# DeepakSridhar/fgdm

Measured on AMD Instinct MI355X. Metric: 512x512 images/sec @ 50 DDIM steps, seg-ControlNet+CFG, higher is better.
Workload: dtype f16

## Files before the change

### fgdm_amd/_lib.py

```python
import ctypes as C
import os

HERE = os.path.dirname(os.path.abspath(__file__))
LIB_PATH = os.path.join(HERE, 'libfgdm_hip.so')

MAX_LEVELS = 8
MAX_CONTROLNETS = 4

FLAG_USE_ORIGINAL = 1
FLAG_ONLY_MID_CONTROL = 2
FLAG_NO_CONTROL = 4
FLAG_CFG_PAIRS = 8

ACT_NONE, ACT_SILU, ACT_RELU, ACT_GEGLU, ACT_QGELU = 0, 1, 2, 3, 4
OUT_F16, OUT_F32, OUT_F32_NCHW, OUT_F16_T = 0, 1, 2, 3
STRIDE2_PAD_BR = -2


class FgdmConfig(C.Structure):
    _fields_ = [
        ('in_channels', C.c_int32), ('out_channels', C.c_int32), ('model_channels', C.c_int32),
        ('num_res_blocks', C.c_int32), ('n_levels', C.c_int32), ('channel_mult', C.c_int32 * MAX_LEVELS),
        ('n_attention_resolutions', C.c_int32), ('attention_resolutions', C.c_int32 * MAX_LEVELS),
        ('num_heads', C.c_int32), ('context_dim', C.c_int32), ('use_adapter', C.c_int32),
# ... 38 lines not shown
    'fgdm_controlnet': (_i, [_p, _i, _p, _p, _p, _i, _i, _i, _p, _i64, _p]),
    'fgdm_ddim_step': (_i, [_p, _p, _p, _f, _f, _f, _f, _f, _p, _p, _p, _p, _i64, _p]),
    'fgdm_plms_combine': (_i, [_p, _p, _p, _p, _i, _p, _i64, _p]),
    'fgdm_axpby': (_i, [_p, _f, _p, _f, _p, _i64, _p]),
    'fgdm_mask_blend': (_i, [_p, _p, _p, _p, _i64, _p]),
    'fgdm_ancestral_step': (_i, [_p, _p, _f, _f, _f, _f, _f, _p, _p, _i64, _p]),
    'fgdm_sample_ddim': (_i, [_p, _p, _p, _p, _f, _i, C.POINTER(_i64), C.POINTER(_f), C.POINTER(_f), C.POINTER(_f),
                              _p, _i, _i, _i, _i, _p]),
    'fgdm_profile_begin': (_i, [_p, _i]),
    'fgdm_profile_end': (_i, [_p, C.POINTER(C.c_double)]),
    'fgdm_workspace_stats': (_i, [_p, C.POINTER(_i64), C.POINTER(_i64)]),
    'fgdm_launch_stats': (_i, [_p, C.POINTER(_i64), C.POINTER(_i64), C.POINTER(_i64)]),
    'fgdm_op_conv2d': (_i, [_p, _i, _p, _i, _p, _p, _p, _p, _i, _i, _i, _i, _i, _i, _i, _i, _f, _p, _p]),
    'fgdm_op_linear': (_i, [_p, _p, _p, _p, _i, _i, _i, _i, _i, _i, _i, _p, _p]),
    'fgdm_debug_force_igemm_cfg': (_i, [_i]),
    'fgdm_bench_igemm': (_i, [_i] * 13 + [C.POINTER(_f)]),
    'fgdm_op_linear_ln_linear': (_i, [_p] * 8 + [_i] * 5 + [_p, _p, C.POINTER(_i), _p]),
    'fgdm_bench_norm': (_i, [_i] * 7 + [C.POINTER(_f)]),
    'fgdm_bench_attention': (_i, [_i] * 6 + [C.POINTER(_f)]),
    'fgdm_bench_ff': (_i, [_i] * 4 + [C.POINTER(_f)]),
    'fgdm_op_groupnorm': (_i, [_p, _i, _p, _i, _i, _i, _p, _p, _f, _i, _p, _p]),
    'fgdm_op_layernorm': (_i, [_p, _i, _i, _p, _p, _f, _p, _p]),
    'fgdm_op_attention': (_i, [_p, _i, _p, _i, _p, _i, _p, _i, _i, _i, _i, _i, _i, _p]),
    'fgdm_op_attention_ex': (_i, [_p, _i, _p, _i, _p, _i, _p, _i, _i, _i, _i, _i, _i, _i, _p]),
    'fgdm_debug_last_attention_kernel': (_i, []),
    'fgdm_op_small_attention': (_i, [_p, _i, _i, _i, _p, _i, _i, _i, _i, _i, _i, _p]),
    'fgdm_op_vae_attention': (_i, [_p, _p, _p, _p, _i, _i, _i, _p]),
    'fgdm_op_softmax_rows': (_i, [_p, _p, _i, _i, _p]),
    'fgdm_op_nchw_to_nhwc': (_i, [_p, _p, _i, _i, _i, _i, _p]),
    'fgdm_op_nhwc_to_nchw': (_i, [_p, _p, _i, _i, _i, _p]),
# ... 29 lines not shown
```

### fgdm_amd/csrc/common.h

```cpp
#pragma once
#include <hip/hip_runtime.h>
#include <stdint.h>

typedef _Float16 half_t;
typedef _Float16 h8 __attribute__((ext_vector_type(8)));
typedef _Float16 h4 __attribute__((ext_vector_type(4)));
typedef _Float16 h2 __attribute__((ext_vector_type(2)));
typedef float f32x16 __attribute__((ext_vector_type(16)));
typedef float f32x4 __attribute__((ext_vector_type(4)));

__device__ __forceinline__ float gelu_f(float x) {
    const float z = fminf(fabsf(x), 6.0f);
    float p = -4.7132482596e-04f;
    p = __builtin_fmaf(p, z, 7.0652551839e-03f);
    p = __builtin_fmaf(p, z, -5.1762067461e-02f);
    p = __builtin_fmaf(p, z, -4.6008771426e-01f);
    p = __builtin_fmaf(p, z, -1.1507295505e+00f);
    p = __builtin_fmaf(p, z, -4.8959157159e-05f - 1.0f);
    const float t = __builtin_amdgcn_exp2f(p);
    return __builtin_fmaf(fabsf(x), 0.5f - t, 0.5f * x);
}

typedef float f32x2 __attribute__((ext_vector_type(2)));
__device__ __forceinline__ f32x2 gelu2_f(f32x2 x) {
// ... 34 lines not shown
    void* out;
    const half_t* zero;
    int C0, C1;
    int B, H, W;
    int Ho, Wo;
    int M, N;
    int K;
    int mode, act, out_kind;
    int ld_out, ld_res;
    int rv_stride;
    int rows_per_sample;
    float scale;
    int force_cfg;
    int splitk;
    float* ws;
    int debug;
    const float* ln_stats;
    const float* ln_u;
    int ln_slots;
    float ln_eps;
    float* stats_out;
    void* out2;
    int split_n, out_kind2, ld_out2;
};

int igemm_launch(const IgemmArgs& a, hipStream_t s);
void igemm_set_force_cfg(int cfg);
void igemm_set_twin_layers(bool on);
void igemm_set_pair_hint(int mult);
int igemm2_launch(const IgemmArgs& a, int cfg, hipStream_t s);
int igemm_stats_slots(const IgemmArgs& a);
int row_stats_slots(int C);
int row_stats_launch(const half_t* x, int rows, int C, float* stats , hipStream_t s);
int igemm_splitk_factor(const IgemmArgs& a);
int igemm_splitk_reduce(const IgemmArgs& a, hipStream_t s);
size_t igemm_npad(int n);

#define GN_PIX_PER_CHUNK 256
void groupnorm_set_group(bool on);
int groupnorm_launch(const half_t* x0, int C0, const half_t* x1, int C1, int B, int HW,
                     const float* gamma, const float* beta, float eps, int silu,
                     half_t* out, float* ws , hipStream_t s);
size_t groupnorm_ws_floats(int B, int HW);
int layernorm_launch(const half_t* x, int rows, int C, const float* gamma, const float* beta, float eps,
                     half_t* out, hipStream_t s);

int attention_launch(const half_t* Q, int ldq, const half_t* K, int ldk, const half_t* Vt, int ldvt,
                     half_t* O, int ldo, int B, int H, int T, int Tk, int d, int q_prescaled, hipStream_t s);
int attention_last_kernel();

// ... 71 lines not shown
```

### fgdm_amd/csrc/engine.hip

```cpp
#include "engine_shared.h"
#include "knobs.h"

#include <algorithm>
#include <array>
#include <cmath>
#include <cstdlib>
#include <cstdio>
#include <cstring>
#include <map>
#include <memory>
#include <string>
#include <unordered_map>
#include <vector>

namespace {

struct Arena {
    struct Blk { char* p; size_t sz; bool free; };
    std::vector<std::vector<Blk>> slabs;
    std::vector<char*> bases;
    size_t slab_bytes = (size_t)4 << 30;
    size_t in_use = 0, peak = 0;
    bool scoped = false;
    std::vector<void*> live;
// ... 240 lines not shown
    std::unordered_map<std::string, ParamSlot> params;
    Net unet;
    std::vector<Net> cns;
    Vae vae;
    Clip clip;
    struct CtxKV { Tensor k, vt; };
    std::unordered_map<const Layer*, CtxKV> ctx_cache;
    int ctx_B = 0, ctx_T = 0;
    int ctx_tokens = 77;
    Arena arena;
    half_t* zero = nullptr;
    std::unordered_map<std::string, std::vector<void*>> weight_allocs;
    std::unordered_map<std::string, bool> comp_dirty, comp_packed;
    std::string cur_comp;
    bool ln_fold = true;
    hipStream_t s = nullptr;
    std::vector<std::unique_ptr<Arena>> cn_arena;
    Arena* ar = &arena;
    hipStream_t s2 = nullptr;
    hipEvent_t ev_fork = nullptr, ev_join = nullptr;
    bool twin_streams = false;
    bool pair_launch = true;
    int group_max = FGDM_MAX_GROUP;
    bool gn_group = true;
    long paired_launches = 0, replayed_launches = 0, paired_problems = 0;
    struct Deferred { const GemmW* w; Tensor src; int idx; float scale; Arena* owner; };
    Prof prof;

    int fail(int code, const std::string& m) { err = m; return code; }

// ... 656 lines not shown
        a.mode = mode; a.act = e.act; a.out_kind = e.out_kind;
        const int nout = e.act == ACT_GEGLU ? w.N / 2 : w.N;
        a.out = e.out ? e.out : (void*)out->p;
        a.ld_out = e.ld_out ? e.ld_out : nout;
        a.rows_per_sample = e.rps ? e.rps : Ho * Wo;
        a.scale = e.scale;
        a.out2 = e.out2; a.out_kind2 = e.out_kind2; a.ld_out2 = e.ld_out2; a.split_n = e.split_n;
        const int taps = mode == IG_LINEAR ? 1 : 9;
        if (taps * (a.C0 + a.C1) != a.K) return fail(FGDM_ERR_ARG, "gemm: K mismatch");
        if (!a.out) return fail(FGDM_ERR_NOMEM, "gemm: null output (workspace exhausted?)");
        char tag[56] = "";
        if (prof.on) snprintf(tag, sizeof(tag), "igemm M%d N%d K%d mode%d act%d out%d l%ds%dr%dv%d", a.M, a.N, a.K, a.mode, a.act, a.out_kind,
                              e.ln ? 1 : 0, e.stats ? 1 : 0, e.resid ? 1 : 0, e.rowvec ? 1 : 0);
        a.splitk = igemm_splitk_factor(a);
        if (a.splitk > 1) {
            a.ws = (float*)ar->alloc((size_t)a.splitk * a.M * a.N * sizeof(float));
            if (!a.ws) return fail(FGDM_ERR_NOMEM, "workspace (split-K partials)");
        }
        if (e.ln) {
            if (!w.ln_u || !e.ln->p || a.splitk > 1) return fail(FGDM_ERR_STATE, "gemm: LayerNorm fold without folded weights / statistics");
            a.ln_stats = e.ln->p; a.ln_slots = e.ln->slots; a.ln_u = w.ln_u; a.ln_eps = w.ln_eps;
        } else if (w.ln_u) {
            return fail(FGDM_ERR_STATE, "gemm: these weights have a LayerNorm folded in; statistics are required");
        }
        if (e.stats) {
            e.stats->slots = igemm_stats_slots(a);
            e.stats->p = (float*)ar->alloc((size_t)a.M * std::max(e.stats->slots, row_stats_slots(nout)) * 2 * sizeof(float));
            if (!e.stats->p) return fail(FGDM_ERR_NOMEM, "workspace (LayerNorm statistics)");
            if (e.stats->slots) a.stats_out = e.stats->p;
        }
        double nbytes = 0.0;
// ... 993 lines not shown
    for (auto& a : e->cn_arena) a->end_scope(rc != FGDM_OK);
    return rc;
}

extern "C" {

static std::string g_create_err;

int fgdm_create(const fgdm_config* cfg, int device, fgdm_engine** out) {
    if (!cfg || !out) return FGDM_ERR_ARG;
    fgdm_engine* e = nullptr;
    int rc = make_desc(cfg, &e);
    if (rc != FGDM_OK) { g_create_err = "unsupported configuration"; return rc; }
    e->device = device;
    e->ln_fold = knob_on(KNOB_LN_FOLD);
    rc = e->ensure_device();
    if (rc != FGDM_OK) {
        g_create_err = e->err + " [" + hipGetErrorString(hipGetLastError()) + "]";
        delete e;
        return rc;
    }
    e->twin_streams = knob_on(KNOB_TWIN_STREAMS);
    e->pair_launch = knob_on(KNOB_PAIR_LAUNCH);
    e->group_max = std::max(2, std::min(FGDM_MAX_GROUP, knob_int(KNOB_GROUP_MAX)));
    e->gn_group = knob_on(KNOB_GN_GROUP);
    if (e->twin_streams && !e->cns.empty()) {
        if (hipStreamCreateWithFlags(&e->s2, hipStreamNonBlocking) != hipSuccess ||
            hipEventCreateWithFlags(&e->ev_fork, hipEventDisableTiming) != hipSuccess ||
            hipEventCreateWithFlags(&e->ev_join, hipEventDisableTiming) != hipSuccess) {
            g_create_err = "second stream could not be created";
// ... 318 lines not shown
```

### fgdm_amd/csrc/engine_shared.h

```cpp
#pragma once
#include "common.h"
#include "../../include/fgdm.h"

#include <algorithm>
#include <cmath>
#include <vector>

static int roundup(int x, int m) { return (x + m - 1) / m * m; }

static std::vector<int> conv3_kmap(int Cin, int* cin_pad) {
    const bool implicit = (Cin % 64) == 0;
    const int cp = implicit ? Cin : roundup(Cin, Cin % 8 == 0 ? 8 : 4);
    const int K = implicit ? 9 * Cin : roundup(9 * cp, 64);
    std::vector<int> kmap(K, -1);
    for (int tap = 0; tap < 9; ++tap)
        for (int c = 0; c < Cin; ++c) {
            const int k = implicit ? ((c >> 6) * 9 + tap) * 64 + (c & 63) : tap * cp + c;
            kmap[k] = c * 9 + tap;
        }
    *cin_pad = cp;
    return kmap;
}

template <class After, class Gemm>
// ... 27 lines not shown
    ~TmpDev() { for (void* p : ptrs) (void)hipFree(p); }
    template <typename T> T* alloc(size_t n) {
        T* d = nullptr;
        if (hipMalloc(&d, n * sizeof(T)) != hipSuccess) return nullptr;
        ptrs.push_back(d);
        return d;
    }
    template <typename T> T* up(const std::vector<T>& h) {
        T* d = alloc<T>(std::max<size_t>(h.size(), 256 / sizeof(T)));
        if (d) (void)hipMemcpy(d, h.data(), h.size() * sizeof(T), hipMemcpyHostToDevice);
        return d;
    }
};
static int plan_splitk(IgemmArgs& a, TmpDev& tmp) {
    a.splitk = igemm_splitk_factor(a);
    if (a.splitk > 1 && !(a.ws = tmp.alloc<float>((size_t)a.splitk * a.M * a.N))) return FGDM_ERR_NOMEM;
    return FGDM_OK;
}
inline half_t* g_zero_page() {
    static half_t* z = nullptr;
    if (!z) { if (hipMalloc(&z, 4096) != hipSuccess) return nullptr; (void)hipMemset(z, 0, 4096); }
    return z;
}
```

### fgdm_amd/csrc/igemm.hip

```cpp
#include "common.h"
#include "knobs.h"
#include <algorithm>

#define LDS_AS __attribute__((address_space(3)))
#define GLB_AS __attribute__((address_space(1)))

__device__ __forceinline__ void glds16(const void* g, void* lds_wave_base) {
    __builtin_amdgcn_global_load_lds((const GLB_AS void*)g, (LDS_AS void*)lds_wave_base, 16, 0, 0);
}


__device__ __forceinline__ float ln_scale(float acc, float mean, float rstd, float u) {
    float t, w;
    asm("v_fma_f32 %0, %1, %2, %3" : "=v"(t) : "v"(-mean), "v"(u), "v"(acc));
    asm("v_mul_f32 %0, %1, %2" : "=v"(w) : "v"(rstd), "v"(t));
    return w;
}

template <int BM, int BN, int WM, int WN>
__global__ __launch_bounds__(WM * WN * 64) void igemm_kernel(const IgemmArgs a) {
    constexpr int T = WM * WN * 64;
    constexpr int TM = BM / WM, TN = BN / WN;
    constexpr int MI = TM / 32, NI = TN / 32;
    constexpr int A_IT = BM * 8 / T, B_IT = BN * 8 / T;
// ... 291 lines not shown
            else if (a.N == 128 && rows >= 192) force = 10;
        }
    }
    return force;
}

int igemm_stats_slots(const IgemmArgs& a) {
    if (a.out_kind != OUT_F16 || a.act == ACT_GEGLU || a.splitk > 1 || (a.N % 320) || (a.K & 31) || (a.C0 & 31) || (a.C1 & 31)) return 0;
    const int f = pick_force(a);
    if (f < 4) return 0;
    const int tile = (f - 4) & 15;
    const bool stats64 = knob_once(KNOB_IGEMM_STATS64) != 0;
    return (tile == 0 || tile == 2 || tile == 3 || tile == 5 || (tile == 7 && stats64)) ? a.N / 160 : 0;
}

int igemm_launch(const IgemmArgs& a, hipStream_t s) {
    if (a.M <= 0 || a.N <= 0 || a.K <= 0 || (a.K & 63) || (a.C0 & 63) || (a.C1 & 63)) return FGDM_ERR_ARG;
    if (a.act == ACT_GEGLU && (a.N & 63)) return FGDM_ERR_ARG;
    if (a.ln_stats && (a.mode != IG_LINEAR || a.C1 || a.ln_slots <= 0 || !a.ln_u)) return FGDM_ERR_ARG;
    if (a.stats_out && igemm_stats_slots(a) == 0) return FGDM_ERR_ARG;
    if (a.out2 && (a.act == ACT_GEGLU || a.splitk > 1 || a.stats_out || a.split_n <= 0 || a.split_n >= a.N || (a.split_n % 640))) return FGDM_ERR_ARG;
    if (a.splitk > 1) {
        if (!a.ws || a.ln_stats) return FGDM_ERR_ARG;
        const bool fat = (long)((a.M + 255) / 256) * (a.N / 320) * a.splitk >= 192 && !(a.K & 31) && !(a.C0 & 31) && !(a.C1 & 31);
        const int rc = igemm2_launch(a, fat ? 0 : 2, s);
        return rc == FGDM_OK ? igemm_splitk_reduce(a, s) : rc;
    }
    int force = pick_force(a);
    const bool mfma32 = knob_once(KNOB_IGEMM_MFMA32) != 0;
    if (mfma32 && force >= 4 && force <= 6 && !a.force_cfg && !g_force_cfg) force += 3;
    if (force >= 4) return igemm2_launch(a, force - 4, s);
    struct Cfg { int bm, bn; float eff; int per_cu; };
    static const Cfg cfgs[] = {{128, 128, 1.00f, 2}, {128, 64, 0.80f, 3}, {64, 64, 0.62f, 4}};
    int best = 0;
    float best_cost = 1e30f;
    for (int i = 0; i < 3; ++i) {
        const Cfg& c = cfgs[i];
        const long nblk = (long)((a.M + c.bm - 1) / c.bm) * ((a.N + c.bn - 1) / c.bn);
        const long slots = 256L * c.per_cu;
        const float rounds = (float)((nblk + slots - 1) / slots);
        const long conc = std::min<long>(c.per_cu, (nblk + 255) / 256);
// ... 13 lines not shown
```

### fgdm_amd/csrc/igemm2.hip

```cpp
#include "common.h"
#include "knobs.h"
#include <algorithm>
#include <type_traits>

#pragma clang diagnostic ignored "-Winline-asm"
#define LDS_AS __attribute__((address_space(3)))
#define GLB_AS __attribute__((address_space(1)))

namespace {

__device__ __forceinline__ void glds16(const void* g, unsigned lds_wave_addr) {
    unsigned keep;
    asm volatile("s_mov_b32 %0, m0\n\ts_mov_b32 m0, %2\n\ts_nop 0\n\tglobal_load_lds_dwordx4 %1, off\n\ts_mov_b32 m0, %0"
                 : "=&s"(keep)
                 : "v"(g), "s"(lds_wave_addr)
                 : "memory", "m0");
}
__device__ __forceinline__ void glds16_m0(const void* g, unsigned lds_wave_addr) {
    asm volatile("s_mov_b32 m0, %1\n\ts_nop 0\n\tglobal_load_lds_dwordx4 %0, off" ::"v"(g), "s"(lds_wave_addr) : "memory", "m0");
}
__device__ __forceinline__ void glds16_sv(unsigned voff, const void* sbase, unsigned lds_wave_addr) {
    asm volatile("s_mov_b32 m0, %2\n\ts_nop 0\n\tglobal_load_lds_dwordx4 %0, %1" ::"v"(voff), "s"(sbase), "s"(lds_wave_addr) : "memory", "m0");
}
__device__ __forceinline__ unsigned lds_addr(const void* p) { return (unsigned)(size_t)(LDS_AS const void*)p; }
// ... 479 lines not shown
            step(std::true_type{}, kt + 1, xb, xa);
        }
        if (kt < nr) {
            step(std::true_type{}, kt, xa, xb);
            ++kt;
#pragma unroll
            for (int i = 0; i < MI; ++i) xa[i] = xb[i];
        }
        if (kt < nk) step(std::false_type{}, kt, xa, xb);
        if (kt + 1 < nk) step(std::false_type{}, kt + 1, xb, xa);
        if (kt + 2 < nk) step(std::false_type{}, kt + 2, xa, xb);
        wait_vmcnt<0>();
    }

    if constexpr (SPLIT) {
        float* wsp = a.ws + (size_t)split * a.M * a.N;
#pragma unroll
        for (int i = 0; i < MI; ++i) {
            const int row = m0 + wm * TM + i * MS + lrow;
            if (row >= a.M) continue;
#pragma unroll
            for (int j = 0; j < NI; ++j)
#pragma unroll
                for (int g = 0; g < AR / 4; ++g) {
                    const int col = n0 + wn * TN + j * MS + (MS == 32 ? 8 * g : 0) + lq;
                    f32x4 pk = {acc[j][i][g * 4], acc[j][i][g * 4 + 1], acc[j][i][g * 4 + 2], acc[j][i][g * 4 + 3]};
                    *(f32x4*)(wsp + (size_t)row * a.N + col) = pk;
                }
        }
        return;
// ... 516 lines not shown
        const bool staged = LN && a.out_kind2 == OUT_F16_T && a.rows_per_sample % 32 == 0 && a.M % 32 == 0 && a.ld_out2 % 8 == 0 &&
                            ((size_t)a.out2 & 15) == 0;
        if (!staged || a.rowvec) return 0;
    }
    if (!a.rowvec) return 1;
    return (BM - 1) / a.rows_per_sample + 2 <= RV_MAX ? 2 : 0;
}
template <int BM, int BN, int WM, int WN, int STAGES, bool CONV, bool GEGLU, bool SPLIT, int MS, bool LN, bool FAST, int PIPE>
int launch2(const IgemmArgs& a, hipStream_t s) {
    const bool fast_on = knob_once(KNOB_IGEMM_EPI_PATHS) != 0;
    if constexpr (FAST && !SPLIT && !LN) {
        if (a.debug)
            return epilogue_path<BM, GEGLU, LN>(a) == 1 ? launch2p<BM, BN, WM, WN, STAGES, CONV, GEGLU, SPLIT, MS, LN, 1, (PIPE == 2 ? 1 : PIPE), true>(a, s)
                                                        : FGDM_ERR_ARG;
    }
    if (a.debug) return FGDM_ERR_ARG;
    if constexpr (SPLIT) return launch2p<BM, BN, WM, WN, STAGES, CONV, GEGLU, SPLIT, MS, LN, 0, PIPE, false>(a, s);
    if constexpr (FAST && !SPLIT) {
        switch (fast_on ? epilogue_path<BM, GEGLU, LN>(a) : 0) {
            case 1: return launch2p<BM, BN, WM, WN, STAGES, CONV, GEGLU, SPLIT, MS, LN, 1, PIPE, false>(a, s);
            case 2: if constexpr (!GEGLU && !LN) return launch2p<BM, BN, WM, WN, STAGES, CONV, GEGLU, SPLIT, MS, LN, 2, PIPE, false>(a, s);
            default: break;
        }
    }
    return launch2p<BM, BN, WM, WN, STAGES, CONV, GEGLU, SPLIT, MS, LN, 0, 0, false>(a, s);
}
template <int BM, int BN, bool GEGLU, int MS, int PIPE, int WM, int WN>
int launch2m(const IgemmArgs& a, hipStream_t s) {
    constexpr int PL = PIPE == 2 ? 1 : PIPE;
    return a.mode == IG_LINEAR ? launch2<BM, BN, WM, WN, 4, false, GEGLU, false, MS, false, MS == 16, PL>(a, s)
// ... 3 lines not shown
int launch2ln(const IgemmArgs& a, hipStream_t s) {
    return launch2<BM, BN, WM, WN, 4, false, GEGLU, false, MS, true, MS == 16, (PIPE == 2 ? 1 : PIPE)>(a, s);
}
template <int BM, int BN, int MS, int PIPE, int WM = 4, int WN = 2>
int launch_tile(const IgemmArgs& a, hipStream_t s) {
    const bool g = a.act == ACT_GEGLU;
    if (a.ln_stats) {
        if constexpr (BN == 256) { if (g) return launch2ln<BM, BN, true, MS, PIPE, WM, WN>(a, s); }
        if constexpr (BN == 128) return FGDM_ERR_ARG;
        else return launch2ln<BM, BN, false, MS, PIPE, WM, WN>(a, s);
    }
    if constexpr (BN == 256) { if (g) return launch2m<BM, BN, true, MS, PIPE, WM, WN>(a, s); }
    return launch2m<BM, BN, false, MS, PIPE, WM, WN>(a, s);
}

__global__ __launch_bounds__(256) void splitk_reduce_kernel(const IgemmArgs a) {
    const size_t total4 = (size_t)a.M * a.N / 4, plane = (size_t)a.M * a.N;
    for (size_t i = (size_t)blockIdx.x * 256 + threadIdx.x; i < total4; i += (size_t)gridDim.x * 256) {
        const size_t e0 = i * 4;
        const int row = (int)(e0 / a.N), col = (int)(e0 - (size_t)row * a.N);
        f32x4 v = *(const f32x4*)(a.ws + e0);
        for (int s = 1; s < a.splitk; ++s) {
            const f32x4 u = *(const f32x4*)(a.ws + (size_t)s * plane + e0);
            v[0] += u[0]; v[1] += u[1]; v[2] += u[2]; v[3] += u[3];
        }
        h4 r = {(half_t)0, (half_t)0, (half_t)0, (half_t)0};
        if (a.resid) r = *(const h4*)(a.resid + (size_t)row * a.ld_res + col);
        h4 o;
#pragma unroll
        for (int e = 0; e < 4; ++e) {
            float x = v[e] + (a.bias ? a.bias[col + e] : 0.f);
            if (a.rowvec) x += a.rowvec[(size_t)(row / a.rows_per_sample) * a.rv_stride + col + e];
            if (a.act == ACT_SILU) x = silu_f(x);
            else if (a.act == ACT_RELU) x = fmaxf(x, 0.f);
            else if (a.act == ACT_QGELU) x = silu_f(x, 1.702f);
            const half_t y = (half_t)(x * a.scale);
            o[e] = a.resid ? (half_t)((float)y + (float)r[e]) : y;
        }
        *(h4*)((half_t*)a.out + (size_t)row * a.ld_out + col) = o;
    }
}

}

static thread_local bool g_twin_layers = false;
void igemm_set_twin_layers(bool on) { g_twin_layers = on; }

int igemm_splitk_factor(const IgemmArgs& a) {
    if (a.force_cfg || a.act == ACT_GEGLU || a.out_kind != OUT_F16 || a.N % 320 || (a.K & 31)) return 1;
    const int nk = a.K >> 5;
    const bool fat = knob_once(KNOB_SPLITK_FAT) != 0;
    if (fat && a.rows_per_sample > 64 && a.rows_per_sample <= 256 && (nk >= 540 || (nk >= 360 && !g_twin_layers))) return 2;
    if (a.rows_per_sample > 64 || nk < 96) return 1;
    return (fat && nk >= 360) ? 8 : 4;
}
int igemm_splitk_reduce(const IgemmArgs& a, hipStream_t s) {
    const size_t total4 = (size_t)a.M * a.N / 4;
    const int grid = (int)std::min<size_t>(2048, (total4 + 255) / 256);
    FGDM_LAUNCH(splitk_reduce_kernel, dim3(grid), dim3(256), 0, s, a);
    return hipGetLastError() == hipSuccess ? FGDM_OK : FGDM_ERR_HIP;
}

static bool halo_geometry(const IgemmArgs& a) {
    if (a.mode != IG_CONV3 || a.Ho != a.H || a.Wo != a.W || (a.C0 & 63) || (a.C1 & 63) || (a.K % 288) || a.debug) return false;
    if ((a.W == 16 || a.W == 32 || a.W == 64) && (a.H * a.W) % 256 == 0) return true;
    return a.W == 8 && a.H == 8;
}

int igemm2_launch(const IgemmArgs& a, int cfg, hipStream_t s) {
    if ((a.K & 31) || (a.C0 & 31) || (a.C1 & 31)) return FGDM_ERR_ARG;
    const int pipe_default = knob_once(KNOB_IGEMM_PIPE);
    const int tile = cfg & 15, psel = cfg >> 4;
    const size_t px = a.mode == IG_LINEAR ? (size_t)a.M : (size_t)a.B * a.H * a.W;
    const bool small = px * (size_t)std::max(a.C0, a.C1) * 2 < (1ull << 32) && (size_t)(a.N + 320) * a.K * 2 < (1ull << 32);
    const bool pipe = (psel == 0 ? pipe_default != 0 : psel == 2) && small;
    const bool halo = knob_once(KNOB_IGEMM_HALO) != 0 && pipe && halo_geometry(a);
    const int bn = (tile == 1 || tile == 4) ? 256 : tile == 6 ? 128 : tile == 7 ? 160 : 320;
    if (a.N % bn) return FGDM_ERR_ARG;
    if (a.act == ACT_GEGLU && bn != 256) return FGDM_ERR_ARG;
    if (a.splitk > 1) {
        if ((tile != 2 && tile != 0) || a.ln_stats) return FGDM_ERR_ARG;
        const int nk_all = a.K >> 5;
        if (halo && nk_all % a.splitk == 0 && (nk_all / a.splitk) % 9 == 0)
            return tile == 0 ? launch2<256, 320, 4, 2, 4, true, false, true, 16, false, false, 2>(a, s)
                             : launch2<128, 320, 4, 2, 4, true, false, true, 16, false, false, 2>(a, s);
        if (tile == 0 && pipe)
            return a.mode == IG_LINEAR ? launch2<256, 320, 4, 2, 4, false, false, true, 16, false, false, 1>(a, s)
                                       : launch2<256, 320, 4, 2, 4, true, false, true, 16, false, false, 1>(a, s);
        if (pipe)
            return a.mode == IG_LINEAR ? launch2<128, 320, 4, 2, 4, false, false, true, 16, false, false, 1>(a, s)
                                       : launch2<128, 320, 4, 2, 4, true, false, true, 16, false, false, 1>(a, s);
        return a.mode == IG_LINEAR ? launch2<128, 320, 4, 2, 4, false, false, true, 16, false, false, 0>(a, s)
                                   : launch2<128, 320, 4, 2, 4, true, false, true, 16, false, false, 0>(a, s);
    }
    if (a.ln_stats && a.mode != IG_LINEAR) return FGDM_ERR_ARG;
    const int persist_mode = knob_once(KNOB_IGEMM_PERSIST);
    const bool persist_on = persist_mode != 0;
    if (persist_on && tile == 1 && pipe && a.act == ACT_GEGLU && a.mode == IG_LINEAR && !a.C1 && a.out_kind == OUT_F16 && !a.rowvec &&
// ... 17 lines not shown
```

### fgdm_amd/csrc/knobs.h

```cpp
#pragma once
#include "common.h"
#include <array>
#include <cstdlib>

#define FGDM_STR_(x) #x
#define FGDM_STR(x) FGDM_STR_(x)

#define FGDM_KNOBS(X)                                                                                                          \
    X(ATTN_PP, "FGDM_ATTN_PP", "1", "0: the four-wave attention kernel where the eight-wave ping-pong one would run")           \
    X(ATTN_DQ, "FGDM_ATTN_DQ", "3", "long self-attention, d = 40: 3 = two-strand kernel, 32-wide V^T P^T; 1 = 16-wide; 0 = off") \
    X(ATTN_DQ80, "FGDM_ATTN_DQ80", "1", "0: the ping-pong kernel instead of the two-strand one at d = 80")                      \
    X(ATTN_ABL, "FGDM_ATTN_ABL", "0", "ablation instantiations of the two-strand kernel (tools/bench_attention.py only)")       \
    X(ATTN_CROSS, "FGDM_ATTN_CROSS", "4", "query chunks per wave of the text-token kernel (65 - 96 keys); 0 = off")             \
    X(ATTN_CROSS_LONG, "FGDM_ATTN_CROSS_LONG", "8", "query chunks per wave of the key-resident kernel (97 - 256 keys); 0 = off") \
    X(IGEMM_EPI_PATHS, "FGDM_IGEMM_EPI_PATHS", "1", "0: the general GEMM epilogue instead of the host-selected straight-line paths") \
    X(IGEMM_HALO, "FGDM_IGEMM_HALO", "1", "0: per-tap K loop instead of the halo-tile loop (stride-1 3x3 convolutions, split K too)") \
    X(IGEMM_MFMA32, "FGDM_IGEMM_MFMA32", "0", "1: automatic tile choices take the 32x32x16 MFMA instantiations")                \
    X(IGEMM_OTHER_WIDTHS, "FGDM_IGEMM_OTHER_WIDTHS", "1", "0: widths 128 / 256 / 512 back on the 2-stage kernel")               \
    X(IGEMM_PERSIST, "FGDM_IGEMM_PERSIST", "1", "GEGLU projections: 1 = persistent, tiles round-robin; 2 = contiguous runs; 0 = off") \
    X(IGEMM_PIPE, "FGDM_IGEMM_PIPE", "1", "0: the phase-locked K loop instead of the software-pipelined one")                   \
    X(IGEMM_SMALL_M, "FGDM_IGEMM_SMALL_M", "1", "0: linears with a thin 128-row grid stay on 128 x 320 tiles")                  \
    X(IGEMM_SMALL_TILES, "FGDM_IGEMM_SMALL_TILES", "1", "0: the 8x8 level's linears back on the 2-stage kernel")                \
    X(IGEMM_STATS64, "FGDM_IGEMM_STATS64", "1", "0: the 64 x 160 tile leaves the LayerNorm partial sums to the row-statistics pass") \
    X(SPLITK_FAT, "FGDM_SPLITK_FAT", "1", "0: split K four ways on 128 x 320 tiles at the 8x8 level only")                      \
    X(PAIR_FAT_TILES, "FGDM_PAIR_FAT_TILES", "1", "0: grouped launches keep the tile a single problem would take")              \
    X(GN_REG, "FGDM_GN_REG", "1024", "largest pixel count per sample of the register-resident GroupNorm; 0 = off")              \
    X(GN_REG_NG, "FGDM_GN_REG_NG", "4", "widest slice of the register-resident GroupNorm, in groups")                           \
    X(GN_FUSED_MAXKB, "FGDM_GN_FUSED_MAXKB", "64", "largest LDS slice (KB) of the single-kernel GroupNorm; 0 = always two kernels") \
    X(GN_CHUNK, "FGDM_GN_CHUNK", FGDM_STR(GN_PIX_PER_CHUNK), "pixels per partial-sum chunk of the two-kernel GroupNorm (multiples of 64)") \
    X(LN_FOLD, "FGDM_LN_FOLD", "1", "fgdm_create; 0: the transformer blocks' LayerNorms as kernels of their own")               \
    X(TWIN_STREAMS, "FGDM_TWIN_STREAMS", "0", "fgdm_create; 1: the ControlNets on a second stream next to the UNet encoder")    \
    X(PAIR_LAUNCH, "FGDM_PAIR_LAUNCH", "1", "fgdm_create; 0: no grouped launches of twin layers")                               \
    X(GROUP_MAX, "FGDM_GROUP_MAX", FGDM_STR(FGDM_MAX_GROUP), "fgdm_create; problems per grouped launch, clamped to [2, FGDM_MAX_GROUP]") \
    X(GN_GROUP, "FGDM_GN_GROUP", "1", "fgdm_create; 0: single-pass GroupNorm launches stay out of the grouped launches")        \
    X(PAIR_DEBUG, "FGDM_PAIR_DEBUG", nullptr, "set (to anything): fgdm_destroy prints how many replayed launches were fused")   \
    X(PROF_DUMP, "FGDM_PROF_DUMP", nullptr, "path: fgdm_profile_end writes the per-shape time table there")                     \
    X(BENCH_DATA_SCALE, "FGDM_BENCH_DATA_SCALE", "1", "atof; scale of the random operands of fgdm_bench_igemm / _attention")

enum Knob {
// ... 28 lines not shown
```

### fgdm_amd/csrc/ops_abi.hip

```cpp
#include "engine_shared.h"

static int op_pack(IgemmArgs& a, TmpDev& tmp, const float* w, const float* bias, int N, int K, int Ks, bool geglu,
                   const int* kmap = nullptr, const float* gamma = nullptr, const float* beta = nullptr) {
    auto host = [](const float* d, size_t n, std::vector<float>& v) { v.resize(n); return hipMemcpy(v.data(), d, n * sizeof(float), hipMemcpyDefault) == hipSuccess; };
    std::vector<float> wh, bh(N, 0.f), g, bt;
    if (!host(w, (size_t)N * Ks, wh) || (bias && !host(bias, N, bh))) return FGDM_ERR_HIP;
    if (gamma && (!host(gamma, K, g) || !host(beta, K, bt))) return FGDM_ERR_HIP;
    const size_t npad = igemm_npad(N);
    std::vector<half_t> pk(npad * (size_t)K, (half_t)0);
    std::vector<float> bp(npad, 0.f), u(gamma ? npad : 0, 0.f);
    for (int pr = 0; pr < N; ++pr) {
        int sr = pr;
        if (geglu) { const int grp = pr >> 6, within = pr & 63; sr = within < 32 ? grp * 32 + within : N / 2 + grp * 32 + (within - 32); }
        const float* row = &wh[(size_t)sr * Ks];
        double us = 0.0, cs = 0.0;
        for (int k = 0; k < K; ++k) {
            const int ks = kmap ? kmap[k] : k;
            if (ks < 0) continue;
            const half_t wq = (half_t)(gamma ? row[ks] * g[k] : row[ks]);
            pk[(size_t)pr * K + k] = wq;
            if (gamma) { us += (double)(float)wq; cs += (double)bt[k] * (double)row[ks]; }
        }
        bp[pr] = gamma ? (float)((double)bh[sr] + cs) : bh[sr];
        if (gamma) u[pr] = (float)us;
// ... 123 lines not shown
    rc = igemm_launch(a, s);
    if (rc == FGDM_OK && !slots) { slots = row_stats_slots(C); rc = row_stats_launch((const half_t*)h_out, M, C, stats, s); }
    if (slots_used) *slots_used = a.stats_out ? slots : -slots;
    if (rc != FGDM_OK) { (void)hipStreamSynchronize(s); return rc; }
    b.A0 = (const half_t*)h_out; b.C0 = C; b.zero = a.zero;
    b.ln_stats = stats; b.ln_slots = slots; b.ln_eps = 1e-5f;
    const int nout = act2 == ACT_GEGLU ? N2 / 2 : N2;
    b.B = 1; b.H = 1; b.W = M; b.Ho = 1; b.Wo = M; b.M = M; b.N = N2; b.K = C; b.mode = IG_LINEAR; b.act = act2;
    b.out_kind = OUT_F16; b.out = y_out; b.ld_out = nout; b.rows_per_sample = M; b.scale = 1.f;
    rc = igemm_launch(b, s);
    (void)hipStreamSynchronize(s);
    return rc;
}

int fgdm_debug_force_igemm_cfg(int cfg) { igemm_set_force_cfg(cfg); return FGDM_OK; }

int fgdm_op_groupnorm(const void* x0, int C0, const void* x1, int C1, int B, int HW, const float* gamma, const float* beta,
                      float eps, int silu, void* out, void* stream) {
    if (!x0 || !gamma || !beta || !out) return FGDM_ERR_ARG;
    hipStream_t s = as_stream(stream);
    float* ws = nullptr;
    if (hipMalloc(&ws, groupnorm_ws_floats(B, HW) * sizeof(float)) != hipSuccess) return FGDM_ERR_NOMEM;
    const int rc = groupnorm_launch((const half_t*)x0, C0, (const half_t*)x1, C1, B, HW, gamma, beta, eps, silu, (half_t*)out, ws, s);
    (void)hipStreamSynchronize(s);
    (void)hipFree(ws);
    return rc;
}
int fgdm_op_layernorm(const void* x, int rows, int C, const float* gamma, const float* beta, float eps, void* out, void* stream) {
    if (!x || !gamma || !beta || !out) return FGDM_ERR_ARG;
    return layernorm_launch((const half_t*)x, rows, C, gamma, beta, eps, (half_t*)out, as_stream(stream));
// ... 67 lines not shown
```

### include/fgdm.h

```cpp
#ifndef FGDM_H
#define FGDM_H
#include <stdint.h>
#ifdef __cplusplus
extern "C" {
#endif

#define FGDM_MAX_LEVELS 8
#define FGDM_MAX_CONTROLNETS 4

typedef struct fgdm_engine fgdm_engine;

typedef struct fgdm_config {
    int32_t in_channels, out_channels, model_channels, num_res_blocks;
    int32_t n_levels;
    int32_t channel_mult[FGDM_MAX_LEVELS];
    int32_t n_attention_resolutions;
    int32_t attention_resolutions[FGDM_MAX_LEVELS];
    int32_t num_heads, context_dim;
    int32_t use_adapter;
    int32_t n_controlnets;
    int32_t hint_channels;
    int64_t workspace_bytes;
    int32_t vae_ch, vae_n_levels;
    int32_t vae_ch_mult[FGDM_MAX_LEVELS];
// ... 69 lines not shown
int fgdm_profile_begin(fgdm_engine* e, int stride );
int fgdm_profile_end(fgdm_engine* e, double* out);
int fgdm_workspace_stats(fgdm_engine* e, int64_t* peak_bytes, int64_t* reserved_bytes);
int fgdm_launch_stats(fgdm_engine* e, int64_t* replayed_launches, int64_t* fused_launches, int64_t* fused_problems);

#define FGDM_STRIDE2_PAD_BR (-2)
int fgdm_op_conv2d(const void* x0, int C0, const void* x1, int C1, const float* w, const float* bias,
                   const float* rowvec, const void* resid, int B, int H, int W, int Cout, int ksize, int stride,
                   int upsample, int act, float scale, void* out, void* stream);
int fgdm_op_linear(const void* x, const float* w, const float* bias, const void* resid, int M, int K, int N,
                   int act, int out_kind, int rows_per_sample, int ld_out, void* out, void* stream);
int fgdm_op_linear_ln_linear(const void* x, const float* w1, const float* b1, const void* resid, const float* gamma,
                             const float* beta, const float* w2, const float* b2, int M, int K1, int C, int N2, int act2,
                             void* h_out, void* y_out, int* slots_used, void* stream);
int fgdm_debug_force_igemm_cfg(int cfg);
int fgdm_bench_igemm(int B, int H, int W, int C0, int C1, int Cout, int ksize, int stride, int upsample, int act,
                     int use_resid, int cfg, int iters, float* avg_ms);
int fgdm_bench_ff(int M, int C, int chunk_rows, int iters, float* avg_ms);
int fgdm_bench_attention(int B, int heads, int T, int Tk, int d, int iters, float* avg_ms);
int fgdm_bench_norm(int kind, int B, int HW, int C0, int C1, int silu, int iters, float* avg_ms);
int fgdm_op_groupnorm(const void* x0, int C0, const void* x1, int C1, int B, int HW, const float* gamma,
                      const float* beta, float eps, int silu, void* out, void* stream);
int fgdm_op_layernorm(const void* x, int rows, int C, const float* gamma, const float* beta, float eps,
                      void* out, void* stream);
int fgdm_op_attention(const void* q, int ldq, const void* k, int ldk, const void* vt, int ldvt, void* o, int ldo,
                      int B, int heads, int T, int Tk, int d, void* stream);
int fgdm_op_attention_ex(const void* q, int ldq, const void* k, int ldk, const void* vt, int ldvt, void* o, int ldo,
                         int B, int heads, int T, int Tk, int d, int q_prescaled, void* stream);
int fgdm_debug_last_attention_kernel(void);
int fgdm_op_small_attention(const void* qkv, int ld, int koff, int voff, void* out, int ldo, int B, int heads, int T, int d,
// ... 16 lines not shown
```

Measured before the change: 7.835.

## Store split-K partials tile-major in MFMA fragment order with a tiled reduce

Split-K GEMM partial sums are now written in tile-major, fragment-native order, so each lane stores contiguous float4 values instead of scattered row-major ones. A new reduce kernel reads these planes and specialises on the split factor so all partial loads can be issued together before the bias, activation and residual epilogue. This targets the uncoalesced partial stores and the reduce pass's memory traffic. The workspace is padded to whole 256-row tiles, and the change adds a knob plus debug hooks for the last split-K configuration.

Result: no change. 7.847, median of 6 (+0.1%).

```diff
diff --git a/fgdm_amd/_lib.py b/fgdm_amd/_lib.py
--- a/fgdm_amd/_lib.py
+++ b/fgdm_amd/_lib.py
@@ -76,6 +76,7 @@
     'fgdm_op_conv2d': (_i, [_p, _i, _p, _i, _p, _p, _p, _p, _i, _i, _i, _i, _i, _i, _i, _i, _f, _p, _p]),
     'fgdm_op_linear': (_i, [_p, _p, _p, _p, _i, _i, _i, _i, _i, _i, _i, _p, _p]),
     'fgdm_debug_force_igemm_cfg': (_i, [_i]),
+    'fgdm_debug_last_splitk': (_i, []),
     'fgdm_bench_igemm': (_i, [_i] * 13 + [C.POINTER(_f)]),
     'fgdm_op_linear_ln_linear': (_i, [_p] * 8 + [_i] * 5 + [_p, _p, C.POINTER(_i), _p]),
     'fgdm_bench_norm': (_i, [_i] * 7 + [C.POINTER(_f)]),
diff --git a/fgdm_amd/csrc/common.h b/fgdm_amd/csrc/common.h
--- a/fgdm_amd/csrc/common.h
+++ b/fgdm_amd/csrc/common.h
@@ -72,6 +72,7 @@
     int force_cfg;
     int splitk;
     float* ws;
+    int ws_tiled;
     int debug;
     const float* ln_stats;
     const float* ln_u;
@@ -91,7 +92,10 @@
 int row_stats_slots(int C);
 int row_stats_launch(const half_t* x, int rows, int C, float* stats , hipStream_t s);
 int igemm_splitk_factor(const IgemmArgs& a);
-int igemm_splitk_reduce(const IgemmArgs& a, hipStream_t s);
+size_t igemm_splitk_ws_floats(const IgemmArgs& a);
+int igemm_splitk_reduce(const IgemmArgs& a, int bm, hipStream_t s);
+bool igemm2_split_halo(const IgemmArgs& a);
+int igemm_last_splitk();
 size_t igemm_npad(int n);
 
 #define GN_PIX_PER_CHUNK 256
diff --git a/fgdm_amd/csrc/engine.hip b/fgdm_amd/csrc/engine.hip
--- a/fgdm_amd/csrc/engine.hip
+++ b/fgdm_amd/csrc/engine.hip
@@ -278,6 +278,7 @@
     std::unordered_map<std::string, bool> comp_dirty, comp_packed;
     std::string cur_comp;
     bool ln_fold = true;
+    bool splitk_tiled = true;
     hipStream_t s = nullptr;
     std::vector<std::unique_ptr<Arena>> cn_arena;
     Arena* ar = &arena;
@@ -964,7 +965,8 @@
                               e.ln ? 1 : 0, e.stats ? 1 : 0, e.resid ? 1 : 0, e.rowvec ? 1 : 0);
         a.splitk = igemm_splitk_factor(a);
         if (a.splitk > 1) {
-            a.ws = (float*)ar->alloc((size_t)a.splitk * a.M * a.N * sizeof(float));
+            a.ws_tiled = splitk_tiled ? 1 : 0;
+            a.ws = (float*)ar->alloc(igemm_splitk_ws_floats(a) * sizeof(float));
             if (!a.ws) return fail(FGDM_ERR_NOMEM, "workspace (split-K partials)");
         }
         if (e.ln) {
@@ -1988,6 +1990,7 @@
     if (rc != FGDM_OK) { g_create_err = "unsupported configuration"; return rc; }
     e->device = device;
     e->ln_fold = knob_on(KNOB_LN_FOLD);
+    e->splitk_tiled = knob_on(KNOB_SPLITK_PLANES);
     rc = e->ensure_device();
     if (rc != FGDM_OK) {
         g_create_err = e->err + " [" + hipGetErrorString(hipGetLastError()) + "]";
diff --git a/fgdm_amd/csrc/engine_shared.h b/fgdm_amd/csrc/engine_shared.h
--- a/fgdm_amd/csrc/engine_shared.h
+++ b/fgdm_amd/csrc/engine_shared.h
@@ -1,5 +1,6 @@
 #pragma once
 #include "common.h"
+#include "knobs.h"
 #include "../../include/fgdm.h"
 
 #include <algorithm>
@@ -65,7 +66,8 @@
 };
 static int plan_splitk(IgemmArgs& a, TmpDev& tmp) {
     a.splitk = igemm_splitk_factor(a);
-    if (a.splitk > 1 && !(a.ws = tmp.alloc<float>((size_t)a.splitk * a.M * a.N))) return FGDM_ERR_NOMEM;
+    a.ws_tiled = knob_on(KNOB_SPLITK_PLANES) ? 1 : 0;
+    if (a.splitk > 1 && !(a.ws = tmp.alloc<float>(igemm_splitk_ws_floats(a)))) return FGDM_ERR_NOMEM;
     return FGDM_OK;
 }
 inline half_t* g_zero_page() {
diff --git a/fgdm_amd/csrc/igemm.hip b/fgdm_amd/csrc/igemm.hip
--- a/fgdm_amd/csrc/igemm.hip
+++ b/fgdm_amd/csrc/igemm.hip
@@ -329,7 +329,11 @@
     return (tile == 0 || tile == 2 || tile == 3 || tile == 5 || (tile == 7 && stats64)) ? a.N / 160 : 0;
 }
 
+static int g_last_splitk = 0;
+int igemm_last_splitk() { return g_last_splitk; }
+
 int igemm_launch(const IgemmArgs& a, hipStream_t s) {
+    g_last_splitk = 0;
     if (a.M <= 0 || a.N <= 0 || a.K <= 0 || (a.K & 63) || (a.C0 & 63) || (a.C1 & 63)) return FGDM_ERR_ARG;
     if (a.act == ACT_GEGLU && (a.N & 63)) return FGDM_ERR_ARG;
     if (a.ln_stats && (a.mode != IG_LINEAR || a.C1 || a.ln_slots <= 0 || !a.ln_u)) return FGDM_ERR_ARG;
@@ -338,8 +342,10 @@
     if (a.splitk > 1) {
         if (!a.ws || a.ln_stats) return FGDM_ERR_ARG;
         const bool fat = (long)((a.M + 255) / 256) * (a.N / 320) * a.splitk >= 192 && !(a.K & 31) && !(a.C0 & 31) && !(a.C1 & 31);
-        const int rc = igemm2_launch(a, fat ? 0 : 2, s);
-        return rc == FGDM_OK ? igemm_splitk_reduce(a, s) : rc;
+        int rc = igemm2_launch(a, fat ? 0 : 2, s);
+        if (rc == FGDM_OK) rc = igemm_splitk_reduce(a, fat ? 256 : 128, s);
+        if (rc == FGDM_OK) g_last_splitk = a.splitk | (fat ? 16 : 0) | (igemm2_split_halo(a) ? 32 : 0) | (a.ws_tiled ? 64 : 0);
+        return rc;
     }
     int force = pick_force(a);
     const bool mfma32 = knob_once(KNOB_IGEMM_MFMA32) != 0;
diff --git a/fgdm_amd/csrc/igemm2.hip b/fgdm_amd/csrc/igemm2.hip
--- a/fgdm_amd/csrc/igemm2.hip
+++ b/fgdm_amd/csrc/igemm2.hip
@@ -517,6 +517,33 @@
     }
 
     if constexpr (SPLIT) {
+        if constexpr (ABL) {
+            if (a.debug & 4) {
+                float sink = 0.f;
+#pragma unroll
+                for (int j = 0; j < NI; ++j)
+#pragma unroll
+                    for (int i = 0; i < MI; ++i) sink += acc[j][i][0] + acc[j][i][AR - 1];
+                if (sink == 12345.678f) a.ws[0] = sink;
+                return;
+            }
+        }
+        if (a.ws_tiled) {
+            static_assert(MS == 16 && AR == 4, "fragment order of the 16x16x32 MFMA");
+            const int ntm = (a.M + BM - 1) / BM;
+            unsigned lz = 0;
+            asm volatile("" : "+v"(lz));
+            const int ln = (int)__builtin_amdgcn_mbcnt_hi(~0u, __builtin_amdgcn_mbcnt_lo(~0u, lz));
+            float* wst = a.ws + (((size_t)split * ntm + m0 / BM) * ntn + n0 / BN) * (size_t)(BM * BN) + (wave * (MI * NI * 64) + ln) * 4;
+#pragma unroll
+            for (int i = 0; i < MI; ++i)
+#pragma unroll
+                for (int j = 0; j < NI; ++j) {
+                    f32x4 pk = {acc[j][i][0], acc[j][i][1], acc[j][i][2], acc[j][i][3]};
+                    *(f32x4*)(wst + (i * NI + j) * 256) = pk;
+                }
+            return;
+        }
         float* wsp = a.ws + (size_t)split * a.M * a.N;
 #pragma unroll
         for (int i = 0; i < MI; ++i) {
@@ -1063,6 +1090,9 @@
             return epilogue_path<BM, GEGLU, LN>(a) == 1 ? launch2p<BM, BN, WM, WN, STAGES, CONV, GEGLU, SPLIT, MS, LN, 1, (PIPE == 2 ? 1 : PIPE), true>(a, s)
                                                         : FGDM_ERR_ARG;
     }
+    if constexpr (SPLIT && CONV && BM == 256 && PIPE == 1) {
+        if (a.debug) return (a.debug & ~12) ? FGDM_ERR_ARG : launch2p<BM, BN, WM, WN, STAGES, CONV, GEGLU, SPLIT, MS, LN, 0, 1, true>(a, s);
+    }
     if (a.debug) return FGDM_ERR_ARG;
     if constexpr (SPLIT) return launch2p<BM, BN, WM, WN, STAGES, CONV, GEGLU, SPLIT, MS, LN, 0, PIPE, false>(a, s);
     if constexpr (FAST && !SPLIT) {
@@ -1096,6 +1126,22 @@
     return launch2m<BM, BN, false, MS, PIPE, WM, WN>(a, s);
 }
 
+__device__ __forceinline__ void splitk_finish(const IgemmArgs& a, const f32x4 v, int row, int col) {
+    h4 r = {(half_t)0, (half_t)0, (half_t)0, (half_t)0};
+    if (a.resid) r = *(const h4*)(a.resid + (size_t)row * a.ld_res + col);
+    h4 o;
+#pragma unroll
+    for (int e = 0; e < 4; ++e) {
+        float x = v[e] + (a.bias ? a.bias[col + e] : 0.f);
+        if (a.rowvec) x += a.rowvec[(size_t)(row / a.rows_per_sample) * a.rv_stride + col + e];
+        if (a.act == ACT_SILU) x = silu_f(x);
+        else if (a.act == ACT_RELU) x = fmaxf(x, 0.f);
+        else if (a.act == ACT_QGELU) x = silu_f(x, 1.702f);
+        const half_t y = (half_t)(x * a.scale);
+        o[e] = a.resid ? (half_t)((float)y + (float)r[e]) : y;
+    }
+    *(h4*)((half_t*)a.out + (size_t)row * a.ld_out + col) = o;
+}
 __global__ __launch_bounds__(256) void splitk_reduce_kernel(const IgemmArgs a) {
     const size_t total4 = (size_t)a.M * a.N / 4, plane = (size_t)a.M * a.N;
     for (size_t i = (size_t)blockIdx.x * 256 + threadIdx.x; i < total4; i += (size_t)gridDim.x * 256) {
@@ -1106,21 +1152,68 @@
             const f32x4 u = *(const f32x4*)(a.ws + (size_t)s * plane + e0);
             v[0] += u[0]; v[1] += u[1]; v[2] += u[2]; v[3] += u[3];
         }
-        h4 r = {(half_t)0, (half_t)0, (half_t)0, (half_t)0};
-        if (a.resid) r = *(const h4*)(a.resid + (size_t)row * a.ld_res + col);
-        h4 o;
-#pragma unroll
-        for (int e = 0; e < 4; ++e) {
-            float x = v[e] + (a.bias ? a.bias[col + e] : 0.f);
-            if (a.rowvec) x += a.rowvec[(size_t)(row / a.rows_per_sample) * a.rv_stride + col + e];
-            if (a.act == ACT_SILU) x = silu_f(x);
-            else if (a.act == ACT_RELU) x = fmaxf(x, 0.f);
-            else if (a.act == ACT_QGELU) x = silu_f(x, 1.702f);
-            const half_t y = (half_t)(x * a.scale);
-            o[e] = a.resid ? (half_t)((float)y + (float)r[e]) : y;
-        }
-        *(h4*)((half_t*)a.out + (size_t)row * a.ld_out + col) = o;
-    }
+        splitk_finish(a, v, row, col);
+    }
+}
+template <int BM, int S>
+__global__ __launch_bounds__(256) void splitk_reduce_tiled_kernel(const IgemmArgs a) {
+    constexpr int BN = 320, WN = 2, TM = BM / 4, TN = BN / WN, MI = TM / 16, NI = TN / 16;
+    constexpr int QW = MI * NI * 64, QT = 8 * QW;
+    constexpr int U = 2, CH = QT / (256 * U);
+    static_assert(QW % 256 == 0 && QT % (256 * U) == 0, "a workgroup's quads lie in one wave tile");
+    const int ntn = a.N / BN, ntm = (a.M + BM - 1) / BM;
+    const int tile = blockIdx.x / CH, chunk = blockIdx.x - tile * CH;
+    const int tm = tile / ntn, tn = tile - tm * ntn;
+    const size_t plane = (size_t)ntm * ntn * (BM * BN);
+    const int nsplit = S ? S : a.splitk;
+    const float* base = a.ws + (size_t)tile * (BM * BN);
+    int row[U], col[U], q[U];
+    f32x4 v[U];
+#pragma unroll
+    for (int u = 0; u < U; ++u) {
+        q[u] = (chunk * U + u) * 256 + threadIdx.x;
+        const int wv = q[u] / QW, r = q[u] - wv * QW, fq = r >> 6, lane = r & 63, i = fq / NI, j = fq - i * NI;
+        row[u] = tm * BM + (wv / WN) * TM + i * 16 + (lane & 15);
+        col[u] = tn * BN + (wv % WN) * TN + j * 16 + 4 * (lane >> 4);
+    }
+    if constexpr (S != 0) {
+        f32x4 p[S][U];
+#pragma unroll
+        for (int s = 0; s < S; ++s)
+#pragma unroll
+            for (int u = 0; u < U; ++u)
+                if (row[u] < a.M) p[s][u] = *(const f32x4*)(base + (size_t)s * plane + (size_t)q[u] * 4);
+#pragma unroll
+        for (int u = 0; u < U; ++u) {
+            v[u] = p[0][u];
+#pragma unroll
+            for (int s = 1; s < S; ++s) { v[u][0] += p[s][u][0]; v[u][1] += p[s][u][1]; v[u][2] += p[s][u][2]; v[u][3] += p[s][u][3]; }
+        }
+    } else {
+#pragma unroll
+        for (int u = 0; u < U; ++u) {
+            if (row[u] >= a.M) continue;
+            v[u] = *(const f32x4*)(base + (size_t)q[u] * 4);
+            for (int s = 1; s < nsplit; ++s) {
+                const f32x4 w = *(const f32x4*)(base + (size_t)s * plane + (size_t)q[u] * 4);
+                v[u][0] += w[0]; v[u][1] += w[1]; v[u][2] += w[2]; v[u][3] += w[3];
+            }
+        }
+    }
+#pragma unroll
+    for (int u = 0; u < U; ++u)
+        if (row[u] < a.M) splitk_finish(a, v[u], row[u], col[u]);
+}
+template <int BM>
+int launch_reduce_tiled(const IgemmArgs& a, hipStream_t s) {
+    const int grid = ((a.M + BM - 1) / BM) * (a.N / 320) * (BM * 320 / 4 / 512);
+    switch (a.splitk) {
+        case 2: FGDM_LAUNCH((splitk_reduce_tiled_kernel<BM, 2>), dim3(grid), dim3(256), 0, s, a); break;
+        case 4: FGDM_LAUNCH((splitk_reduce_tiled_kernel<BM, 4>), dim3(grid), dim3(256), 0, s, a); break;
+        case 8: FGDM_LAUNCH((splitk_reduce_tiled_kernel<BM, 8>), dim3(grid), dim3(256), 0, s, a); break;
+        default: FGDM_LAUNCH((splitk_reduce_tiled_kernel<BM, 0>), dim3(grid), dim3(256), 0, s, a); break;
+    }
+    return hipGetLastError() == hipSuccess ? FGDM_OK : FGDM_ERR_HIP;
 }
 
 }
@@ -1136,7 +1229,13 @@
     if (a.rows_per_sample > 64 || nk < 96) return 1;
     return (fat && nk >= 360) ? 8 : 4;
 }
-int igemm_splitk_reduce(const IgemmArgs& a, hipStream_t s) {
+size_t igemm_splitk_ws_floats(const IgemmArgs& a) { return (size_t)a.splitk * (size_t)((a.M + 255) / 256 * 256) * a.N; }
+
+int igemm_splitk_reduce(const IgemmArgs& a, int bm, hipStream_t s) {
+    if (a.ws_tiled) {
+        if (a.N % 320 || (bm != 256 && bm != 128)) return FGDM_ERR_ARG;
+        return bm == 256 ? launch_reduce_tiled<256>(a, s) : launch_reduce_tiled<128>(a, s);
+    }
     const size_t total4 = (size_t)a.M * a.N / 4;
     const int grid = (int)std::min<size_t>(2048, (total4 + 255) / 256);
     FGDM_LAUNCH(splitk_reduce_kernel, dim3(grid), dim3(256), 0, s, a);
@@ -1148,6 +1247,9 @@
     if ((a.W == 16 || a.W == 32 || a.W == 64) && (a.H * a.W) % 256 == 0) return true;
     return a.W == 8 && a.H == 8;
 }
+
+static bool g_split_halo = false;
+bool igemm2_split_halo(const IgemmArgs&) { return g_split_halo; }
 
 int igemm2_launch(const IgemmArgs& a, int cfg, hipStream_t s) {
     if ((a.K & 31) || (a.C0 & 31) || (a.C1 & 31)) return FGDM_ERR_ARG;
@@ -1163,7 +1265,8 @@
     if (a.splitk > 1) {
         if ((tile != 2 && tile != 0) || a.ln_stats) return FGDM_ERR_ARG;
         const int nk_all = a.K >> 5;
-        if (halo && nk_all % a.splitk == 0 && (nk_all / a.splitk) % 9 == 0)
+        g_split_halo = halo && nk_all % a.splitk == 0 && (nk_all / a.splitk) % 9 == 0;
+        if (g_split_halo)
             return tile == 0 ? launch2<256, 320, 4, 2, 4, true, false, true, 16, false, false, 2>(a, s)
                              : launch2<128, 320, 4, 2, 4, true, false, true, 16, false, false, 2>(a, s);
         if (tile == 0 && pipe)
diff --git a/fgdm_amd/csrc/knobs.h b/fgdm_amd/csrc/knobs.h
--- a/fgdm_amd/csrc/knobs.h
+++ b/fgdm_amd/csrc/knobs.h
@@ -23,6 +23,7 @@
     X(IGEMM_SMALL_TILES, "FGDM_IGEMM_SMALL_TILES", "1", "0: the 8x8 level's linears back on the 2-stage kernel")                \
     X(IGEMM_STATS64, "FGDM_IGEMM_STATS64", "1", "0: the 64 x 160 tile leaves the LayerNorm partial sums to the row-statistics pass") \
     X(SPLITK_FAT, "FGDM_SPLITK_FAT", "1", "0: split K four ways on 128 x 320 tiles at the 8x8 level only")                      \
+    X(SPLITK_PLANES, "FGDM_SPLITK_PLANES", "1", "fgdm_create, op / bench entries; 0: row-major split-K partial planes, not tile-major") \
     X(PAIR_FAT_TILES, "FGDM_PAIR_FAT_TILES", "1", "0: grouped launches keep the tile a single problem would take")              \
     X(GN_REG, "FGDM_GN_REG", "1024", "largest pixel count per sample of the register-resident GroupNorm; 0 = off")              \
     X(GN_REG_NG, "FGDM_GN_REG_NG", "4", "widest slice of the register-resident GroupNorm, in groups")                           \
diff --git a/fgdm_amd/csrc/ops_abi.hip b/fgdm_amd/csrc/ops_abi.hip
--- a/fgdm_amd/csrc/ops_abi.hip
+++ b/fgdm_amd/csrc/ops_abi.hip
@@ -161,6 +161,7 @@
 }
 
 int fgdm_debug_force_igemm_cfg(int cfg) { igemm_set_force_cfg(cfg); return FGDM_OK; }
+int fgdm_debug_last_splitk(void) { return igemm_last_splitk(); }
 
 int fgdm_op_groupnorm(const void* x0, int C0, const void* x1, int C1, int B, int HW, const float* gamma, const float* beta,
                       float eps, int silu, void* out, void* stream) {
diff --git a/include/fgdm.h b/include/fgdm.h
--- a/include/fgdm.h
+++ b/include/fgdm.h
@@ -107,6 +107,7 @@
                              const float* beta, const float* w2, const float* b2, int M, int K1, int C, int N2, int act2,
                              void* h_out, void* y_out, int* slots_used, void* stream);
 int fgdm_debug_force_igemm_cfg(int cfg);
+int fgdm_debug_last_splitk(void);
 int fgdm_bench_igemm(int B, int H, int W, int C0, int C1, int Cout, int ksize, int stride, int upsample, int act,
                      int use_resid, int cfg, int iters, float* avg_ms);
 int fgdm_bench_ff(int M, int C, int chunk_rows, int iters, float* avg_ms);
```
